# uc-vision/splat-trainer

Hardware: AMD Instinct MI355X
Metric: fwd+bwd Gaussians/s (higher is better)
Workload: dtype f32

## Files before the change

### include/gsplat_hip.h

```cpp
#ifndef GSPLAT_HIP_H
#define GSPLAT_HIP_H

#include <stddef.h>
#include <stdint.h>

#ifdef __cplusplus
extern "C" {
#endif

#define GSR_OK 0
#define GSR_ERR_INVALID_ARGUMENT -1
#define GSR_ERR_WORKSPACE_TOO_SMALL -2
#define GSR_ERR_LAUNCH_FAILED -3
#define GSR_ERR_UNSUPPORTED -4

#define GSR_ROW_FLOATS 16
#define GSR_PARTIAL_FLOATS 12
#define GSR_MAX_FEATURES 16
#define GSR_WIDE_MIN_FEATURES 4

#ifndef GSR_HAVE_RASTER_PARAMS
#define GSR_HAVE_RASTER_PARAMS
typedef struct GsrRasterParamsC {
  float alpha_threshold;
// ... 110 lines not shown
                                     float* d_position, float* d_log_scaling, float* d_rotation, float* d_alpha_logit,
                                     int32_t mode, float* d_colors_out, float* prune_cost_out, float* split_score_out,
                                     float* visibility_out, float* camera_partials, float* d_camera, void* stream);

int gsr_depth_key_range(float near_plane, float far_plane, uint32_t* bias_out, uint32_t* max_key_out);
int gsr_depth_keys(const float* depth, int64_t M, uint32_t bias, uint32_t max_key, uint32_t* keys_out, void* stream);
int gsr_pack_rows(const float* gaussians2d, const float* depth, const float* features, int64_t M, int32_t C,
                  const GsrRasterParamsC* params_host, float* rows_out, float* screen_scale_out, void* stream);
int gsr_pack_rows_wide(const float* gaussians2d, const float* depth, const float* features, int64_t M, int32_t C,
                       const GsrRasterParamsC* params_host, float* rows_out, float* feat_rows_out, float* screen_scale_out,
                       void* stream);
int gsr_tile_count(const float* rows, const uint32_t* order, int64_t M, int32_t W, int32_t H,
                   const GsrRasterParamsC* params_host, uint32_t* count_out, uint32_t* tile_hits_out,
                   const uint32_t* M_dev , void* stream);
#define GSR_TILE_COUNT_OFFSETS_MAX 4194304
size_t gsr_tile_count_offsets_workspace_bytes(int64_t M);
int gsr_tile_count_offsets(const float* rows, const uint32_t* order, int64_t M, int32_t W, int32_t H,
                           const GsrRasterParamsC* params_host, uint32_t* count_out, uint32_t* tile_hits_out,
                           const uint32_t* M_dev, uint32_t* offsets_out, uint32_t* total_dev, uint32_t* overflow_flag,
                           void* workspace, size_t workspace_bytes, void* stream);
int gsr_tile_emit(const float* rows, const uint32_t* order, const uint32_t* offsets, const uint32_t* tile_hits, int64_t M,
                  int32_t W, int32_t H, const GsrRasterParamsC* params_host, uint32_t* keys_out, uint32_t* inst2splat_out,
                  int64_t capacity, const uint32_t* M_dev , void* stream);
int gsr_tile_ranges(const uint32_t* sorted_keys, int64_t O, int32_t num_tiles, uint32_t* tile_range,
                    const uint32_t* O_dev , void* stream);

int gsr_segment_thresholds(int32_t seg_pairs_cfg, int32_t heavy_min_cfg, int64_t O, int32_t num_tiles, int32_t needs_grad,
                           int32_t* seg_pairs_out, int32_t* heavy_min_out);
int64_t gsr_segment_capacity(int64_t O, int32_t O_is_bound, int32_t seg_pairs_cfg, int32_t heavy_min_cfg, int32_t num_tiles,
                             int32_t needs_grad);
int64_t gsr_segment_heavy_capacity(int64_t O, int32_t O_is_bound, int32_t seg_pairs_cfg, int32_t heavy_min_cfg,
                                   int32_t num_tiles, int32_t needs_grad);
int gsr_segment_plan(const uint32_t* tile_range, int32_t num_tiles, int32_t seg_pairs_cfg, int32_t heavy_min_cfg,
                     int32_t needs_grad, int64_t O, const uint32_t* O_dev, int64_t capacity, int64_t heavy_capacity,
                     uint32_t* tile_seg_out, uint32_t* seg_desc_out, uint32_t* seg_total_out, uint32_t* tile_order_out,
                     void* stream);
int gsr_segment_thresholds_wide(int32_t seg_pairs_cfg, int32_t heavy_min_cfg, int64_t O, int32_t num_tiles,
                                int32_t needs_grad, int32_t wide, int32_t* seg_pairs_out, int32_t* heavy_min_out);
int64_t gsr_segment_capacity_wide(int64_t O, int32_t O_is_bound, int32_t seg_pairs_cfg, int32_t heavy_min_cfg,
                                  int32_t num_tiles, int32_t needs_grad, int32_t wide);
int64_t gsr_segment_heavy_capacity_wide(int64_t O, int32_t O_is_bound, int32_t seg_pairs_cfg, int32_t heavy_min_cfg,
                                        int32_t num_tiles, int32_t needs_grad, int32_t wide);
int gsr_segment_plan_wide(const uint32_t* tile_range, int32_t num_tiles, int32_t seg_pairs_cfg, int32_t heavy_min_cfg,
                          int32_t needs_grad, int32_t wide, int64_t O, const uint32_t* O_dev, int64_t capacity,
                          int64_t heavy_capacity, uint32_t* tile_seg_out, uint32_t* seg_desc_out, uint32_t* seg_total_out,
                          uint32_t* tile_order_out, void* stream);
// ... 56 lines not shown
  const float* rotation_xyzw;
  const float* alpha_logit;
  const float* sh_features;
  int64_t N;
  int32_t K;
  int32_t W, H;
  const float* T_camera_world;
  const float* projection;
  const float* camera_pos;
  float near_plane, far_plane;
  GsrRasterParamsC params;
  int32_t want_jacobian;
  int32_t want_median;
  int32_t compute_visibility;
  int32_t needs_grad;
  int32_t seg_pairs, seg_min_pairs;
  int64_t pair_capacity;
  const float* gaussians2d;
  const float* depth;
  const float* features;
  int32_t C;
  const uint32_t* depth_order;
  int32_t feature_table;
} GsrFrameC;
typedef struct GsrFramePlanC {
  int64_t out_bytes, work_bytes;
  int64_t zero_begin, zero_bytes;
  int64_t prune_cost, split_score, counts, tile_range, vis_partial, indexes, rows, screen_scale, jacobian, visibility,
      image, final_T, last, median, count, offsets, vals_a, vals_b, tvals_a, tvals_b, trank_a, trank_b, pair_vis,
      seg_tables, seg_pix, seg_last;
  int64_t seg_capacity, seg_heavy_capacity;
  int64_t cull_ws, sort_ws, scan_ws, tsort_ws, keys_a, keys_b, tile_hits, tkeys_a, tkeys_b;
  int64_t cull_ws_bytes, sort_ws_bytes, scan_ws_bytes, tsort_ws_bytes;
  int64_t feat_rows;
  int64_t seg_col;
} GsrFramePlanC;
typedef struct GsrFrameResultC {
  int64_t order;
  int64_t sorted_inst;
  int64_t sorted_splat;
  GsrSegmentsC segments;
  int32_t has_segments;
} GsrFrameResultC;
int gsr_frame_plan(const GsrFrameC* frame_host, GsrFramePlanC* plan_out_host);
int gsr_frame_forward(const GsrFrameC* frame_host, const GsrFramePlanC* plan_host, void* out_arena, void* work_arena,
                      GsrFrameResultC* result_out_host, uint32_t* counts_host, void* event_counts, void* event_k6_begin,
// ... 296 lines not shown
```

### splat-trainer_amd/csrc/binning.hip

```cpp
#include "gsr_device.h"
#include "gsr_host.h"

namespace {

inline GsrRasterParams to_params(const GsrRasterParamsC* c) {
  GsrRasterParams rp;
  __builtin_memcpy(&rp, c, sizeof(rp));
  return rp;
}

__global__ __launch_bounds__(256) void depth_keys_kernel(const float* __restrict__ depth, int64_t M,
                                                         uint32_t* __restrict__ keys, uint32_t bias, uint32_t max_key) {
  const int64_t m = (int64_t)blockIdx.x * blockDim.x + threadIdx.x;
  if (m >= M) return;
  keys[m] = gsr_depth_key(depth[m], bias, max_key);
}

struct TileHits {
  uint32_t origin;
  uint32_t shape;
  uint32_t lo, hi;
};

__device__ __forceinline__ uint32_t hits_of_large_extent(float u, float v, float A, float B, float C, float qmax, int x0,
                                                         int x1, int y0, int y1, uint32_t* keys, uint32_t* ranks,
                                                         uint32_t o, uint32_t capacity, uint32_t k, int tiles_x,
                                                         int lane) {
  const int nx = x1 - x0, total = nx * (y1 - y0);
  uint32_t n = 0;
  for (int t0 = 0; t0 < total; t0 += 64) {
    const int t = t0 + lane;
    uint32_t hm = 0u;
    int tx = 0, ty = 0;
    if (t < total) {
      ty = y0 + t / nx;
      tx = x0 + t % nx;
      if (gsr_tile_hit(u, v, A, B, C, qmax, tx, ty)) hm = gsr_tile_half_mask(u, v, A, B, C, qmax, tx, ty);
    }
    const uint64_t hit = __ballot(hm != 0u);
    if (keys && hm) {
      const uint32_t at = o + n + (uint32_t)gsr_mbcnt(hit);
      if (at < capacity) {
        keys[at] = (uint32_t)(ty * tiles_x + tx);
        ranks[at] = k | (hm << 30);
      }
    }
    n += (uint32_t)__builtin_popcountll(hit);
  }
  return n;
}

__device__ __forceinline__ float gsr_bcast(float x, int l) {
  return __int_as_float(__builtin_amdgcn_readlane(__float_as_int(x), l));
}

__device__ __forceinline__ uint32_t wave_large_extents(bool large, float u, float v, float A, float B, float C,
                                                       const GsrExtent& e, uint32_t* keys, uint32_t* ranks, uint32_t o,
                                                       uint32_t capacity, uint32_t sid, int tiles_x, int lane) {
  uint32_t mine = 0u;
  uint64_t todo = __ballot(large);
  while (todo) {
    const int l = __builtin_ctzll(todo);
    todo &= todo - 1ull;
    const uint32_t n = hits_of_large_extent(
        gsr_bcast(u, l), gsr_bcast(v, l), gsr_bcast(A, l), gsr_bcast(B, l), gsr_bcast(C, l), gsr_bcast(e.qmax, l),
        __builtin_amdgcn_readlane(e.x0, l), __builtin_amdgcn_readlane(e.x1, l), __builtin_amdgcn_readlane(e.y0, l),
        __builtin_amdgcn_readlane(e.y1, l), keys, ranks, (uint32_t)__builtin_amdgcn_readlane((int)o, l), capacity,
        (uint32_t)__builtin_amdgcn_readlane((int)sid, l), tiles_x, lane);
    if (lane == l) mine = n;
  }
  return mine;
}

__device__ __forceinline__ uint32_t tile_count_one(const float* __restrict__ rows, uint32_t splat,
                                                   int64_t k, bool live, int tiles_x, int tiles_y,
                                                   const GsrRasterParams& rp, TileHits* __restrict__ hits) {
  float2 uv = make_float2(0.f, 0.f), ab = uv, co = uv;
  GsrExtent e;
  e.x0 = e.x1 = e.y0 = e.y1 = 0; e.qmax = 0.f;
  TileHits h;
  h.origin = 0u; h.shape = 0u; h.lo = 0u; h.hi = 0u;
  uint32_t n = 0;
  bool large = false;
  if (live) {
    const int64_t s = splat;
    const float4* r = reinterpret_cast<const float4*>(rows + GSR_ROW_FLOATS * s);
    const float4 r0 = r[0];
    const float4 r1 = r[1];
    uv = make_float2(r0.x, r0.y); ab = make_float2(r0.z, r0.w); co = make_float2(r1.x, r1.y);
    e = gsr_splat_extent(uv.x, uv.y, ab.x, ab.y, co.x, co.y, rp, tiles_x, tiles_y);
    const int nx = e.x1 - e.x0, ny = e.y1 - e.y0;
    h.origin = (uint32_t)e.x0 | ((uint32_t)e.y0 << 16);
    if (nx > 0 && ny > 0) {
      if (nx * ny <= 32) {
        h.shape = (uint32_t)nx | ((uint32_t)ny << 8);
        uint64_t map = 0ull;
        int t = 0;
        for (int ty = e.y0; ty < e.y1; ++ty)
          for (int tx = e.x0; tx < e.x1; ++tx, ++t) {
            const uint64_t hm = gsr_tile_half_mask(uv.x, uv.y, ab.x, ab.y, co.x, e.qmax, tx, ty);
            map |= hm << (2 * t);
            n += hm ? 1u : 0u;
          }
        h.lo = (uint32_t)map; h.hi = (uint32_t)(map >> 32);
      } else {
        h.shape = 1u << 16;
        large = true;
      }
    }
  }
  const uint32_t nl = wave_large_extents(large, uv.x, uv.y, ab.x, ab.y, co.x, e, nullptr, nullptr, 0u, 0u, 0u, tiles_x,
                                         gsr_lane());
  if (large) n = nl;
  if (live) *reinterpret_cast<uint4*>(hits + k) = make_uint4(h.origin, h.shape, h.lo, h.hi);
  return n;
}

__global__ __launch_bounds__(256) void tile_count_kernel(const float* __restrict__ rows,
                                                         const uint32_t* __restrict__ order, int64_t M, int tiles_x,
                                                         int tiles_y, GsrRasterParams rp, uint32_t* __restrict__ count,
                                                         TileHits* __restrict__ hits,
                                                         const uint32_t* __restrict__ M_dev,
                                                         uint32_t* __restrict__ block_sums) {
// ... 34 lines not shown
  before = gsr_wave_sum_u32(before);
  fbefore = gsr_wave_sum(fbefore + (float)sum);
  if (lane == 63) s_wave[w] = incl;
  if (lane == 0) { s_before[w] = before; s_f[w] = fbefore; }
  __syncthreads();
  uint32_t prefix = (s_before[0] + s_before[1]) + (s_before[2] + s_before[3]), total = 0u;
  uint32_t in_block = 0u;
#pragma unroll
  for (int j = 0; j < 4; ++j) {
    if (j < w) in_block += s_wave[j];
    total += s_wave[j];
  }
  if (threadIdx.x == 0 && (s_f[0] + s_f[1]) + (s_f[2] + s_f[3]) >= 2147000000.f) *overflow = 1u;
  uint32_t run = prefix + in_block + incl - sum;
#pragma unroll
  for (int i = 0; i < 16; ++i) {
    if (base + i < n) offsets[base + i] = run;
    run += v[i];
  }
  if (total_out && blockIdx.x == gridDim.x - 1 && threadIdx.x == 0) *total_out = prefix + total;
}


__global__ __launch_bounds__(256) void tile_emit_kernel(const float* __restrict__ rows,
                                                        const uint32_t* __restrict__ order,
                                                        const uint32_t* __restrict__ offsets,
                                                        const TileHits* __restrict__ hits, int64_t M, int tiles_x,
                                                        int tiles_y, GsrRasterParams rp, uint32_t* __restrict__ keys,
                                                        uint32_t* __restrict__ inst2splat, uint32_t capacity,
                                                        const uint32_t* __restrict__ M_dev) {
  const int64_t k = (int64_t)blockIdx.x * blockDim.x + threadIdx.x;
  const bool live = k < M && !(M_dev && k >= (int64_t)*M_dev);
  uint4 hw = make_uint4(0u, 0u, 0u, 0u);
  uint32_t o = 0u, sid = 0u;
  if (live) {
    hw = *reinterpret_cast<const uint4*>(hits + k);
    o = offsets[k];
    sid = order[k];
  }
  const bool large = (hw.y >> 16) != 0u;
  float4 r0 = make_float4(0.f, 0.f, 0.f, 0.f), r1 = r0;
  GsrExtent e;
  e.x0 = e.x1 = e.y0 = e.y1 = 0; e.qmax = 0.f;
  if (large) {
    const float4* r = reinterpret_cast<const float4*>(rows + GSR_ROW_FLOATS * (int64_t)sid);
    r0 = r[0];
    r1 = r[1];
    e = gsr_splat_extent(r0.x, r0.y, r0.z, r0.w, r1.x, r1.y, rp, tiles_x, tiles_y);
  }
  wave_large_extents(large, r0.x, r0.y, r0.z, r0.w, r1.x, e, keys, inst2splat, o, capacity, sid, tiles_x, gsr_lane());
  if (!live || large) return;
  const int nx = (int)(hw.y & 0xFFu), ny = (int)((hw.y >> 8) & 0xFFu);
  const int x0 = (int)(hw.x & 0xFFFFu), y0 = (int)(hw.x >> 16);
  uint64_t map = (uint64_t)hw.z | ((uint64_t)hw.w << 32);
  for (int j = 0; j < ny; ++j)
    for (int i = 0; i < nx; ++i, map >>= 2) {
      const uint32_t hm = (uint32_t)(map & 3ull);
      if (!hm) continue;
      if (o >= capacity) return;
      keys[o] = (uint32_t)((y0 + j) * tiles_x + x0 + i);
      inst2splat[o] = sid | (hm << 30);
// ... 291 lines not shown
int gsr_tile_count_offsets(const float* rows, const uint32_t* order, int64_t M, int32_t W, int32_t H,
                           const GsrRasterParamsC* params_host, uint32_t* count_out, uint32_t* tile_hits_out,
                           const uint32_t* M_dev, uint32_t* offsets_out, uint32_t* total_dev, uint32_t* overflow_flag,
                           void* workspace, size_t workspace_bytes, void* stream_) {
  hipStream_t stream = gsr_stream(stream_);
  if (M < 0 || M > GSR_TILE_COUNT_OFFSETS_MAX || !params_host || W <= 0 || H <= 0) return GSR_ERR_INVALID_ARGUMENT;
  if (params_host->tile_size != 16) return GSR_ERR_UNSUPPORTED;
  if (!total_dev || !overflow_flag) return GSR_ERR_INVALID_ARGUMENT;
  if (M == 0) { hipMemsetAsync(total_dev, 0, sizeof(uint32_t), stream); return GSR_OK; }
  if (!rows || !order || !count_out || !tile_hits_out || !offsets_out) return GSR_ERR_INVALID_ARGUMENT;
  if (!workspace || workspace_bytes < gsr_tile_count_offsets_workspace_bytes(M)) return GSR_ERR_WORKSPACE_TOO_SMALL;
  const auto [tx, ty, num_tiles] = gsr_tiles(W, H);
  if (tx > 0xFFFF || ty > 0xFFFF) return GSR_ERR_UNSUPPORTED;
  uint32_t* sums = reinterpret_cast<uint32_t*>(workspace);
  tile_count_kernel<<<grid_for(M, 256), 256, 0, stream>>>(rows, order, M, tx, ty, to_params(params_host), count_out,
                                                         reinterpret_cast<TileHits*>(tile_hits_out), M_dev, sums);
  GSR_CHECK_LAUNCH();
  offsets_from_sums_kernel<<<grid_for(M, 4096), 256, 0, stream>>>(count_out, (uint32_t)M, sums, offsets_out, total_dev,
                                                                 overflow_flag);
  GSR_CHECK_LAUNCH();
  return GSR_OK;
}

int gsr_tile_emit(const float* rows, const uint32_t* order, const uint32_t* offsets, const uint32_t* tile_hits, int64_t M,
                  int32_t W, int32_t H, const GsrRasterParamsC* params_host, uint32_t* keys_out, uint32_t* inst2splat_out,
                  int64_t capacity, const uint32_t* M_dev, void* stream_) {
  hipStream_t stream = gsr_stream(stream_);
  if (M < 0 || M >= (1ll << 30) || !params_host || W <= 0 || H <= 0) return GSR_ERR_INVALID_ARGUMENT;
  if (capacity < 0 || capacity > 0x7FFFFFFFll) return GSR_ERR_INVALID_ARGUMENT;
  if (params_host->tile_size != 16) return GSR_ERR_UNSUPPORTED;
  if (M == 0) return GSR_OK;
  if (!rows || !order || !offsets || !tile_hits || !keys_out || !inst2splat_out) return GSR_ERR_INVALID_ARGUMENT;
  const auto [tx, ty, num_tiles] = gsr_tiles(W, H);
  tile_emit_kernel<<<grid_for(M, 256), 256, 0, stream>>>(rows, order, offsets, reinterpret_cast<const TileHits*>(tile_hits),
                                                        M, tx, ty, to_params(params_host), keys_out, inst2splat_out,
                                                        (uint32_t)capacity, M_dev);
  GSR_CHECK_LAUNCH();
  return GSR_OK;
}

int gsr_tile_ranges(const uint32_t* sorted_keys, int64_t O, int32_t num_tiles, uint32_t* tile_range,
                    const uint32_t* O_dev, void* stream_) {
  hipStream_t stream = gsr_stream(stream_);
  if (O < 0 || num_tiles <= 0) return GSR_ERR_INVALID_ARGUMENT;
  if (O == 0) return GSR_OK;
  if (!sorted_keys || !tile_range) return GSR_ERR_INVALID_ARGUMENT;
  tile_ranges_kernel<<<grid_for(O, 256), 256, 0, stream>>>(sorted_keys, O, tile_range, O_dev);
  GSR_CHECK_LAUNCH();
  return GSR_OK;
}

int gsr_reduce_visibility(const float* vis_partial, const uint32_t* offsets, const uint32_t* count,
                          const uint32_t* order, int64_t M, float* visibility_out, int64_t capacity,
                          const uint32_t* M_dev, void* stream_) {
  hipStream_t stream = gsr_stream(stream_);
  if (M < 0 || capacity < 0 || capacity > 0x7FFFFFFFll) return GSR_ERR_INVALID_ARGUMENT;
  if (M == 0) return GSR_OK;
  if (!offsets || !count || !visibility_out) return GSR_ERR_INVALID_ARGUMENT;
  reduce_vis_kernel<<<grid_for(M, 256), 256, 0, stream>>>(vis_partial, offsets, count, order, M, visibility_out,
// ... 52 lines not shown
```

### splat-trainer_amd/csrc/frame.hip

```cpp
#include <string.h>

#include "gsr_host.h"

namespace {

inline int64_t align_up(int64_t x, int64_t a = 256) { return (x + a - 1) / a * a; }

struct Cursor {
  int64_t at = 0;
  int64_t take(int64_t bytes) {
    const int64_t o = at;
    at = align_up(at + (bytes > 0 ? bytes : 1));
    return o;
  }
};

inline int tile_bits_of(int num_tiles) {
  int b = 1;
  while ((1 << b) < num_tiles) ++b;
  return b;
}

inline int bit_length(uint32_t v) {
  int b = 0;
// ... 132 lines not shown
    int64_t* indexes = at<int64_t>(out, p->indexes);
    GSR_TRY(gsr_frustum_cull(f->position, N, f->T_camera_world, f->projection, f->W, f->H, f->near_plane, f->far_plane,
                             f->params.margin_px, indexes, M_dev, at<uint8_t>(work, p->cull_ws),
                             (size_t)p->cull_ws_bytes, stream_));
    GSR_TRY(gsr_project_sh_forward(f->position, f->log_scaling, f->rotation_xyzw, f->alpha_logit, f->sh_features, f->K,
                                   indexes, N, f->T_camera_world, f->projection, f->camera_pos, &f->params, rows,
                                   at<float>(out, p->screen_scale), at<float>(out, p->jacobian), M_dev,
                                   keys_a, key_bias, key_max, stream_));
  }
  uint32_t* vals_a = at<uint32_t>(out, p->vals_a);
  uint32_t* vals_b = at<uint32_t>(out, p->vals_b);
  const uint32_t* order = f->depth_order;
  res->order = -1;
  if (!order) {
    const int in_b = gsr_sort_pairs_u32(keys_a, vals_a, at<uint32_t>(work, p->keys_b), vals_b, N, 1, 0, bit_length(key_max),
                                        at<uint8_t>(work, p->sort_ws), (size_t)p->sort_ws_bytes, M_dev, stream_);
    if (in_b < 0) return in_b;
    res->order = in_b == 1 ? p->vals_b : p->vals_a;
    order = in_b == 1 ? vals_b : vals_a;
  }
  uint32_t* count = at<uint32_t>(out, p->count);
  uint32_t* offsets = at<uint32_t>(out, p->offsets);
  uint32_t* hits = at<uint32_t>(work, p->tile_hits);
  if (N <= GSR_TILE_COUNT_OFFSETS_MAX) {
    GSR_TRY(gsr_tile_count_offsets(rows, order, N, f->W, f->H, &f->params, count, hits, M_dev, offsets, O_dev, counts + 2,
                                   at<uint8_t>(work, p->scan_ws), (size_t)p->scan_ws_bytes, stream_));
  } else {
    GSR_TRY(gsr_tile_count(rows, order, N, f->W, f->H, &f->params, count, hits, M_dev, stream_));
    GSR_TRY(gsr_exclusive_scan_u32_checked(count, offsets, N, O_dev, counts + 2, at<uint8_t>(work, p->scan_ws),
                                           (size_t)p->scan_ws_bytes, stream_));
  }
  if (counts_host) {
    if (hipMemcpyAsync(counts_host, counts, 3 * sizeof(uint32_t), hipMemcpyDeviceToHost, stream) != hipSuccess)
      return GSR_ERR_LAUNCH_FAILED;
    if (event_counts && hipEventRecord(reinterpret_cast<hipEvent_t>(event_counts), stream) != hipSuccess)
      return GSR_ERR_LAUNCH_FAILED;
  }
  res->sorted_inst = res->sorted_splat = -1;
  float* image = at<float>(out, p->image);
  if (cap > 0) {
    uint32_t* tkeys_a = at<uint32_t>(work, p->tkeys_a);
    uint32_t* tkeys_b = at<uint32_t>(work, p->tkeys_b);
    uint32_t* tvals_a = at<uint32_t>(out, p->tvals_a);
    uint32_t* tvals_b = at<uint32_t>(out, p->tvals_b);
    uint32_t* trank_a = at<uint32_t>(out, p->trank_a);
    uint32_t* trank_b = at<uint32_t>(out, p->trank_b);
    GSR_TRY(gsr_tile_emit(rows, order, offsets, hits, N, f->W, f->H, &f->params, tkeys_a, trank_a, cap, M_dev, stream_));
    const int sorted = gsr_sort_pairs2_u32(tkeys_a, tvals_a, trank_a, tkeys_b, tvals_b, trank_b, cap, 1, 0, tile_bits_of(T),
                                           at<uint8_t>(work, p->tsort_ws), (size_t)p->tsort_ws_bytes, O_dev, stream_);
    if (sorted < 0) return sorted;
    const bool in_b = sorted == 1;
    res->sorted_inst = in_b ? p->tvals_b : p->tvals_a;
    res->sorted_splat = in_b ? p->trank_b : p->trank_a;
    const uint32_t* sorted_keys = in_b ? tkeys_b : tkeys_a;
    const uint32_t* sorted_inst = in_b ? tvals_b : tvals_a;
    const uint32_t* sorted_splat = in_b ? trank_b : trank_a;
    uint32_t* tile_range = at<uint32_t>(out, p->tile_range);
    GSR_TRY(gsr_tile_ranges(sorted_keys, cap, T, tile_range, O_dev, stream_));
    const GsrSegmentsC* seg = nullptr;
    if (p->seg_capacity > 0) {
      uint32_t* tables = at<uint32_t>(out, p->seg_tables);
      uint32_t* tile_seg = tables;
      uint32_t* seg_desc = tables + 2 * (int64_t)T + p->seg_heavy_capacity;
      uint32_t* seg_total = counts + 3;
      uint32_t* tile_order = seg_desc + 4 * p->seg_capacity;
      GSR_TRY(gsr_segment_plan_wide(tile_range, T, f->seg_pairs, f->seg_min_pairs, f->needs_grad ? 1 : 0,
                                    p->feat_rows >= 0 ? 1 : 0, cap, O_dev, p->seg_capacity, p->seg_heavy_capacity,
                                    tile_seg, seg_desc, seg_total, tile_order, stream_));
      float* pix = at<float>(out, p->seg_pix);
      res->segments.tile_seg = tile_seg;
// ... 106 lines not shown
```

### splat-trainer_amd/csrc/gsr_math.h

```cpp
#pragma once
#include <math.h>

#if defined(__HIPCC__)
#define GSR_HD __host__ __device__ __forceinline__
#else
#define GSR_HD inline
#endif

struct GsrRasterParams {
  float alpha_threshold;
  float clamp_max_alpha;
  float T_eps;
  float q_max;
  float blur;
  int   antialias;
  int   tile_size;
  float margin_px;
};

struct GsrCam {
  float R[9];
  float t[3];
  float fx, fy, cx, cy;
};
// ... 337 lines not shown
GSR_HD GsrExtent gsr_splat_extent(float u, float v, float A, float B, float C, float op,
                                  const GsrRasterParams& rp, int tiles_x, int tiles_y) {
  GsrExtent e;
  e.x0 = e.x1 = e.y0 = e.y1 = 0;
  e.qmax = 0.f;
  if (!(op >= rp.alpha_threshold)) return e;
  float qop = 2.f * logf(op / rp.alpha_threshold) * 1.0001f + 1e-4f;
  float qmax = fminf(rp.q_max * 1.00001f, qop);
  float det = A * C - B * B;
  if (!(det > 0.f)) return e;
  float hx = sqrtf(qmax * C / det) + 1e-3f;
  float hy = sqrtf(qmax * A / det) + 1e-3f;
  const float ts = 16.f;
  float fx0 = floorf((u - hx - 0.5f) / ts), fx1 = floorf((u + hx - 0.5f) / ts) + 1.f;
  float fy0 = floorf((v - hy - 0.5f) / ts), fy1 = floorf((v + hy - 0.5f) / ts) + 1.f;
  e.x0 = (int)fminf(fmaxf(fx0, 0.f), (float)tiles_x);
  e.x1 = (int)fminf(fmaxf(fx1, 0.f), (float)tiles_x);
  e.y0 = (int)fminf(fmaxf(fy0, 0.f), (float)tiles_y);
  e.y1 = (int)fminf(fmaxf(fy1, 0.f), (float)tiles_y);
  e.qmax = qmax;
  return e;
}

GSR_HD float gsr_edge_min_q(float Kf, float Bc, float Kv, float d_fixed, float lo, float hi) {
  float d = -Bc * d_fixed / Kv;
  d = fminf(fmaxf(d, lo), hi);
  return Kf * d_fixed * d_fixed + 2.f * Bc * d_fixed * d + Kv * d * d;
}

GSR_HD bool gsr_rect_hit(float A, float B, float C, float qmax, float rx0, float rx1, float ry0, float ry1) {
  if (rx0 <= 0.f && rx1 >= 0.f && ry0 <= 0.f && ry1 >= 0.f) return true;
  float m = gsr_edge_min_q(A, B, C, rx0, ry0, ry1);
  m = fminf(m, gsr_edge_min_q(A, B, C, rx1, ry0, ry1));
  m = fminf(m, gsr_edge_min_q(C, B, A, ry0, rx0, rx1));
  m = fminf(m, gsr_edge_min_q(C, B, A, ry1, rx0, rx1));
  return m <= qmax;
}

GSR_HD bool gsr_tile_hit(float u, float v, float A, float B, float C, float qmax, int tx, int ty) {
  return gsr_rect_hit(A, B, C, qmax, 16.f * tx + 0.5f - u, 16.f * tx + 15.5f - u, 16.f * ty + 0.5f - v,
                      16.f * ty + 15.5f - v);
}

GSR_HD unsigned gsr_tile_half_mask(float u, float v, float A, float B, float C, float qmax, int tx, int ty) {
  const float rx0 = 16.f * tx + 0.5f - u, rx1 = 16.f * tx + 15.5f - u;
  const float ry = 16.f * ty + 0.5f - v;
  unsigned m = gsr_rect_hit(A, B, C, qmax, rx0, rx1, ry, ry + 7.f) ? 1u : 0u;
  m |= gsr_rect_hit(A, B, C, qmax, rx0, rx1, ry + 8.f, ry + 15.f) ? 2u : 0u;
  return m;
}
```

### splat-trainer_amd/csrc/hostmath_shim.cpp

```cpp
#include "hostmath_shim.h"

#include <stdint.h>
#include <string.h>

#include <algorithm>
#include <utility>
#include <vector>

#include "gsr_math.h"
#include "gsr_bilagrid.h"
#include "gsr_neighbours.h"
#include "gsr_visibility.h"
#include "gsr_filter3d.h"
#include "gsr_sh_fit.h"
#include "gsr_controller.h"
#include "gsr_camera_table.h"
#include "gsr_color.h"
#include "gsr_eval.h"
#include "gsr_histogram.h"
#include "gsr_image.h"
#include "gsr_undistort.h"
#include "gsr_relocate.h"
#include "gsr_fusion.h"
#include "gsr_mesh.h"
// ... 55 lines not shown
    mask[i] = gsr_in_view(cam, pos[3 * i], pos[3 * i + 1], pos[3 * i + 2], W, H, near_p, far_p, margin) ? 1 : 0;
}

void hm_sh_basis(int K, int64_t M, const float* dirs, float* Y) {
  for (int64_t m = 0; m < M; ++m) {
    const float* d = dirs + 3 * m;
    float* y = Y + (int64_t)K * m;
    switch (K) {
      case 1: gsr_sh_basis<1>(d[0], d[1], d[2], y); break;
      case 4: gsr_sh_basis<4>(d[0], d[1], d[2], y); break;
      case 9: gsr_sh_basis<9>(d[0], d[1], d[2], y); break;
      default: gsr_sh_basis<16>(d[0], d[1], d[2], y); break;
    }
  }
}

void hm_tile_hits(const void* params, int64_t M, const float* g2d, int tiles_x, int tiles_y, uint8_t* hits) {
  GsrRasterParams rp;
  memcpy(&rp, params, sizeof(rp));
  const int64_t nt = (int64_t)tiles_x * tiles_y;
  for (int64_t m = 0; m < M; ++m) {
    const float* g = g2d + 6 * m;
    GsrExtent e = gsr_splat_extent(g[0], g[1], g[2], g[3], g[4], g[5], rp, tiles_x, tiles_y);
    for (int ty = e.y0; ty < e.y1; ++ty)
      for (int tx = e.x0; tx < e.x1; ++tx)
        if (gsr_tile_hit(g[0], g[1], g[2], g[3], g[4], e.qmax, tx, ty)) hits[m * nt + ty * tiles_x + tx] = 1;
  }
}

void hm_splat_extent(const void* params, int64_t M, const float* g2d, int tiles_x, int tiles_y, int32_t* extent,
                     float* qmax) {
  GsrRasterParams rp;
  memcpy(&rp, params, sizeof(rp));
  for (int64_t m = 0; m < M; ++m) {
    const float* g = g2d + 6 * m;
    GsrExtent e = gsr_splat_extent(g[0], g[1], g[2], g[3], g[4], g[5], rp, tiles_x, tiles_y);
    int32_t* o = extent + 4 * m;
    o[0] = e.x0; o[1] = e.x1; o[2] = e.y0; o[3] = e.y1;
    qmax[m] = e.qmax;
  }
}

void hm_tile_half_masks(const void* params, int64_t M, const float* g2d, int tiles_x, int tiles_y, uint8_t* masks) {
  GsrRasterParams rp;
  memcpy(&rp, params, sizeof(rp));
  const int64_t nt = (int64_t)tiles_x * tiles_y;
  for (int64_t m = 0; m < M; ++m) {
    const float* g = g2d + 6 * m;
    GsrExtent e = gsr_splat_extent(g[0], g[1], g[2], g[3], g[4], g[5], rp, tiles_x, tiles_y);
    const bool large = (e.x1 - e.x0) * (e.y1 - e.y0) > 32;
    for (int ty = e.y0; ty < e.y1; ++ty)
      for (int tx = e.x0; tx < e.x1; ++tx) {
        if (large && !gsr_tile_hit(g[0], g[1], g[2], g[3], g[4], e.qmax, tx, ty)) continue;
        masks[m * nt + ty * tiles_x + tx] = (uint8_t)gsr_tile_half_mask(g[0], g[1], g[2], g[3], g[4], e.qmax, tx, ty);
      }
  }
}

static void hm_bg_cols(const float* grid, int L, int GH, int GW, int cx, int cy, float* cols) {
  for (int q = 0; q < 4; ++q)
    for (int l = 0; l < L; ++l)
      for (int c = 0; c < GSR_BG_CH; ++c)
        cols[(q * L + l) * GSR_BG_CH + c] = grid[((c * L + l) * GH + cy + (q >> 1)) * GW + cx + (q & 1)];
}

void hm_bilagrid_forward(const float* grid, int L, int GH, int GW, const float* rgb, int H, int W, float* out) {
  float cols[4 * 64 * GSR_BG_CH];
  const float inv_2w = 1.f / (2.f * (float)W), inv_2h = 1.f / (2.f * (float)H);
  for (int i = 0; i < H; ++i)
    for (int j = 0; j < W; ++j) {
      const int cx = gsr_bg_cell(j, W, GW), cy = gsr_bg_cell(i, H, GH);
      hm_bg_cols(grid, L, GH, GW, cx, cy, cols);
      const float* p = rgb + 3 * ((int64_t)i * W + j);
      gsr_bg_pixel_fwd(cols, L, gsr_bg_frac(j, cx, W, GW, inv_2w), gsr_bg_frac(i, cy, H, GH, inv_2h), p[0], p[1], p[2],
                       out + 3 * ((int64_t)i * W + j));
    }
}
// ... 935 lines not shown
```

### splat-trainer_amd/renderer.py

```python
from __future__ import annotations

import ctypes as C
import os
import threading
from typing import Optional, Tuple

import torch

from . import _lib
from ._args import f32
from ._lib import current_stream_ptr as _stream, ptr as _ptr
from .data_types import CameraParams, Gaussians3D, RasterConfig, RenderedPoints, Rendering
from . import sh as _sh
from .sh import evaluate_sh_at

ROW_FLOATS = _lib.CONSTANTS["GSR_ROW_FLOATS"]
PARTIAL_FLOATS = _lib.CONSTANTS["GSR_PARTIAL_FLOATS"]
CAMERA_GRAD_FLOATS = 20


class KernelTimer:

  def __init__(self):
    self.events = {}
    self._open = {}
    self._pool = []

  def reserve(self, n: int):
    for _ in range(n):
      e = torch.cuda.Event(enable_timing=True)
      e.record(_lib.current_stream())
      self._pool.append(e)

  def _event(self):
    e = self._pool.pop() if self._pool else torch.cuda.Event(enable_timing=True)
    e.record(_lib.current_stream())
    return e

  def begin(self, name: str):
    self._open[name] = self._event()
# ... 382 lines not shown

def _vis_out(st: _RasterState, live: bool):
  if live and st.compute_visibility and not st.vis_ready:
    st.vis_ready = True
    return st.visibility
  return None


class _RasterFn(torch.autograd.Function):

  @staticmethod
  def forward(ctx, g2d, feats, depth, st: _RasterState, order):
    g, f, d = f32(g2d), f32(feats), f32(depth).reshape(-1)
    if st.M == 0:
      image = _blank_frame(st, g.device)
    else:
      st.order = order
      frame = _lib.GsrFrameC(
          N=st.M, K=1, W=st.W, H=st.H, near_plane=st.near_far[0], far_plane=st.near_far[1], params=st.params,
          want_median=int(st.want_median), compute_visibility=int(st.compute_visibility),
          needs_grad=int(bool(st.needs_grad)), seg_pairs=st.seg_pairs, seg_min_pairs=st.seg_min,
          gaussians2d=g.data_ptr(), depth=d.data_ptr(), features=f.data_ptr(), C=st.C,
          depth_order=order.data_ptr() if order is not None else None,
          feature_table=int(st.C >= _lib.WIDE_MIN_FEATURES))
      _, _, _, image = _run_frame(frame, st, g.device, st.M, projected=True)
    ctx.st = st
    ctx.in_dtypes = (g2d.dtype, feats.dtype)
    return image

  @staticmethod
  def backward(ctx, d_image):
    st: _RasterState = ctx.st
    dev = d_image.device
    live = st.M > 0 and st.O > 0
    alloc = torch.empty if live else torch.zeros
    d_g2d = alloc(st.M, 6, dtype=torch.float32, device=dev)
    d_feat = alloc(st.M, st.C, dtype=torch.float32, device=dev)
    if live:
      wide = st.C >= _lib.WIDE_MIN_FEATURES
      grows = _composite_backward_wide(st, d_image, d_feat, dev) if wide else _composite_backward_rows(st, d_image, dev)
      _lib.call("gsr_unpack_grad_rows", _ptr(st.rows), _ptr(grows), st.M, st.C, _ptr(d_g2d), None if wide else _ptr(d_feat),
                _ptr(st.prune_cost), _ptr(st.split_score), _ptr(_vis_out(st, live)), _stream())
    return d_g2d.to(ctx.in_dtypes[0]), d_feat.to(ctx.in_dtypes[1]), None, None, None


def _arena_view(typed: torch.Tensor, offset: int, shape) -> torch.Tensor:
  if len(shape) == 1:
# ... 70 lines not shown
  return out, plan, M, image


class _FrameFn(torch.autograd.Function):

  @staticmethod
  def forward(ctx, position, log_scaling, rotation, alpha_logit, feature, T, proj, cam_pos, cull_args, st: _RasterState,
              grad_out, sink, want_jac):
    pos, ls, rot, al = f32(position), f32(log_scaling), f32(rotation), f32(alpha_logit)
    sh, cam = f32(feature), f32(cam_pos)
    N, K, dev = pos.shape[0], sh.shape[2], pos.device
    W, H, near, far, margin = cull_args
    if N == 0:
      st.M = 0
      image = _blank_frame(st, dev)
      indexes, jac = torch.empty(0, dtype=torch.int64, device=dev), None
    else:
      frame = _lib.GsrFrameC(
          position=pos.data_ptr(), log_scaling=ls.data_ptr(), rotation_xyzw=rot.data_ptr(), alpha_logit=al.data_ptr(),
          sh_features=sh.data_ptr(), N=N, K=K, W=W, H=H, T_camera_world=T.data_ptr(), projection=proj.data_ptr(),
          camera_pos=cam.data_ptr(), near_plane=near, far_plane=far, params=st.params,
          want_jacobian=int(bool(want_jac and K > 1)), want_median=int(st.want_median),
          compute_visibility=int(st.compute_visibility), needs_grad=int(bool(st.needs_grad)), seg_pairs=st.seg_pairs,
          seg_min_pairs=st.seg_min, C=3)
      out, plan, M, image = _run_frame(frame, st, dev, N, projected=False)
      indexes = _arena_view(out.view(torch.int64), plan.indexes, (M,))
      jac = _arena_view(out.view(torch.float32), plan.jacobian, (M, 9)) if plan.jacobian >= 0 else None
    rows = st.rows
    ctx.save_for_backward(pos, ls, rot, al, sh, indexes, T, proj, cam)
    ctx.set_materialize_grads(False)
    ctx.st, ctx.jac, ctx.grad_out, ctx.sink = st, jac, grad_out, sink
    ctx.in_dtypes = (position.dtype, log_scaling.dtype, rotation.dtype, alpha_logit.dtype, feature.dtype)
    ctx.mark_non_differentiable(indexes)
    return image, rows[:, 0:6], rows[:, 10:11], indexes

  @staticmethod
  def backward(ctx, d_image, d_g2d, d_depth, _d_indexes):
    pos, ls, rot, al, sh, indexes, T, proj, cam = ctx.saved_tensors
    st: _RasterState = ctx.st
    M, N, K, dev = indexes.shape[0], pos.shape[0], sh.shape[2], pos.device
    go, sink = ctx.grad_out, ctx.sink
    collector = sink.collector if sink is not None else None
    nothing = (None,) * 13
    want_cam = ctx.needs_input_grad[5] or ctx.needs_input_grad[6]
    partials = d_camera = None
    want_sh = sink is not None or ctx.needs_input_grad[4]
    geometry, feature = _sh.gradient_destinations("render_gaussians.backward", N, M, K, go, sink, want_feature=want_sh)
# ... 148 lines not shown
```

Baseline: 579.7 million.

## Fuse offset scan into tile emit kernel and precompute conic reciprocals

For frames up to a size threshold, the exclusive-scan offsets are now computed inside the tile emit kernel. Each block sums the preceding blocks' per-block totals and does a block scan, which removes a separate scan pass and its launches. Separately, the tile-hit tests precompute 1/A and 1/C once per splat and reuse the edge argmin across the two half-tile rects, replacing per-tile divisions. The fused scan makes each block do O(blockIdx) reads of the block sums, a quadratic-ish cost that grows with M.

After: 568.4 million. -2.0%, worse.

```diff
diff --git a/include/gsplat_hip.h b/include/gsplat_hip.h
--- a/include/gsplat_hip.h
+++ b/include/gsplat_hip.h
@@ -156,6 +156,12 @@
 int gsr_tile_emit(const float* rows, const uint32_t* order, const uint32_t* offsets, const uint32_t* tile_hits, int64_t M,
                   int32_t W, int32_t H, const GsrRasterParamsC* params_host, uint32_t* keys_out, uint32_t* inst2splat_out,
                   int64_t capacity, const uint32_t* M_dev , void* stream);
+#define GSR_TILE_EMIT_SCAN_MAX 1048576
+int gsr_tile_bin(const float* rows, const uint32_t* order, int64_t M, int32_t W, int32_t H,
+                 const GsrRasterParamsC* params_host, uint32_t* count_out, uint32_t* tile_hits_out, const uint32_t* M_dev,
+                 uint32_t* offsets_out, uint32_t* total_dev, uint32_t* overflow_flag, uint32_t* keys_out,
+                 uint32_t* inst2splat_out, int64_t capacity, int64_t emit_scan_max, void* workspace,
+                 size_t workspace_bytes, void* stream);
 int gsr_tile_ranges(const uint32_t* sorted_keys, int64_t O, int32_t num_tiles, uint32_t* tile_range,
                     const uint32_t* O_dev , void* stream);
 
@@ -258,6 +264,7 @@
   int32_t C;
   const uint32_t* depth_order;
   int32_t feature_table;
+  int32_t emit_scan_max;
 } GsrFrameC;
 typedef struct GsrFramePlanC {
   int64_t out_bytes, work_bytes;
diff --git a/splat-trainer_amd/csrc/binning.hip b/splat-trainer_amd/csrc/binning.hip
--- a/splat-trainer_amd/csrc/binning.hip
+++ b/splat-trainer_amd/csrc/binning.hip
@@ -22,10 +22,10 @@
   uint32_t lo, hi;
 };
 
-__device__ __forceinline__ uint32_t hits_of_large_extent(float u, float v, float A, float B, float C, float qmax, int x0,
-                                                         int x1, int y0, int y1, uint32_t* keys, uint32_t* ranks,
-                                                         uint32_t o, uint32_t capacity, uint32_t k, int tiles_x,
-                                                         int lane) {
+__device__ __forceinline__ uint32_t hits_of_large_extent(float u, float v, float A, float B, float C,
+                                                         const GsrConicRcp& r, float qmax, int x0, int x1, int y0,
+                                                         int y1, uint32_t* keys, uint32_t* ranks, uint32_t o,
+                                                         uint32_t capacity, uint32_t k, int tiles_x, int lane) {
   const int nx = x1 - x0, total = nx * (y1 - y0);
   uint32_t n = 0;
   for (int t0 = 0; t0 < total; t0 += 64) {
@@ -35,7 +35,7 @@
     if (t < total) {
       ty = y0 + t / nx;
       tx = x0 + t % nx;
-      if (gsr_tile_hit(u, v, A, B, C, qmax, tx, ty)) hm = gsr_tile_half_mask(u, v, A, B, C, qmax, tx, ty);
+      if (gsr_tile_hit(u, v, A, B, C, r, qmax, tx, ty)) hm = gsr_tile_half_mask(u, v, A, B, C, r, qmax, tx, ty);
     }
     const uint64_t hit = __ballot(hm != 0u);
     if (keys && hm) {
@@ -62,8 +62,9 @@
   while (todo) {
     const int l = __builtin_ctzll(todo);
     todo &= todo - 1ull;
+    const float Al = gsr_bcast(A, l), Cl = gsr_bcast(C, l);
     const uint32_t n = hits_of_large_extent(
-        gsr_bcast(u, l), gsr_bcast(v, l), gsr_bcast(A, l), gsr_bcast(B, l), gsr_bcast(C, l), gsr_bcast(e.qmax, l),
+        gsr_bcast(u, l), gsr_bcast(v, l), Al, gsr_bcast(B, l), Cl, gsr_conic_rcp(Al, Cl), gsr_bcast(e.qmax, l),
         __builtin_amdgcn_readlane(e.x0, l), __builtin_amdgcn_readlane(e.x1, l), __builtin_amdgcn_readlane(e.y0, l),
         __builtin_amdgcn_readlane(e.y1, l), keys, ranks, (uint32_t)__builtin_amdgcn_readlane((int)o, l), capacity,
         (uint32_t)__builtin_amdgcn_readlane((int)sid, l), tiles_x, lane);
@@ -94,11 +95,12 @@
     if (nx > 0 && ny > 0) {
       if (nx * ny <= 32) {
         h.shape = (uint32_t)nx | ((uint32_t)ny << 8);
+        const GsrConicRcp rc = gsr_conic_rcp(ab.x, co.x);
         uint64_t map = 0ull;
         int t = 0;
         for (int ty = e.y0; ty < e.y1; ++ty)
           for (int tx = e.x0; tx < e.x1; ++tx, ++t) {
-            const uint64_t hm = gsr_tile_half_mask(uv.x, uv.y, ab.x, ab.y, co.x, e.qmax, tx, ty);
+            const uint64_t hm = gsr_tile_half_mask(uv.x, uv.y, ab.x, ab.y, co.x, rc, e.qmax, tx, ty);
             map |= hm << (2 * t);
             n += hm ? 1u : 0u;
           }
@@ -179,21 +181,49 @@
 }
 
 
+template <bool SCAN>
 __global__ __launch_bounds__(256) void tile_emit_kernel(const float* __restrict__ rows,
                                                         const uint32_t* __restrict__ order,
-                                                        const uint32_t* __restrict__ offsets,
+                                                        std::conditional_t<SCAN, uint32_t, const uint32_t>* __restrict__
+                                                            offsets,
                                                         const TileHits* __restrict__ hits, int64_t M, int tiles_x,
                                                         int tiles_y, GsrRasterParams rp, uint32_t* __restrict__ keys,
                                                         uint32_t* __restrict__ inst2splat, uint32_t capacity,
-                                                        const uint32_t* __restrict__ M_dev) {
+                                                        const uint32_t* __restrict__ M_dev,
+                                                        const uint32_t* __restrict__ count,
+                                                        const uint32_t* __restrict__ sums256,
+                                                        uint32_t* __restrict__ total_out,
+                                                        uint32_t* __restrict__ overflow) {
   const int64_t k = (int64_t)blockIdx.x * blockDim.x + threadIdx.x;
   const bool live = k < M && !(M_dev && k >= (int64_t)*M_dev);
   uint4 hw = make_uint4(0u, 0u, 0u, 0u);
   uint32_t o = 0u, sid = 0u;
   if (live) {
     hw = *reinterpret_cast<const uint4*>(hits + k);
-    o = offsets[k];
+    if constexpr (!SCAN) o = offsets[k];
     sid = order[k];
+  }
+  if constexpr (SCAN) {
+    const uint32_t c = k < M ? count[k] : 0u;
+    uint32_t before = 0u;
+    float fbefore = 0.f;
+    for (uint32_t j = threadIdx.x; j < blockIdx.x; j += 256u) {
+      const uint32_t b = sums256[j];
+      before += b;
+      fbefore += (float)b;
+    }
+    before = gsr_wave_sum_u32(before);
+    fbefore = gsr_wave_sum(fbefore + (float)c);
+    const auto front = gsr_block_handoff(before, fbefore);
+    const uint32_t prefix = (front.a[0] + front.a[1]) + (front.a[2] + front.a[3]);
+    const float shadow = (front.b[0] + front.b[1]) + (front.b[2] + front.b[3]);
+    uint32_t total;
+    o = prefix + gsr_block_scan_excl(c, &total);
+    if (k < M) offsets[k] = o;
+    if (threadIdx.x == 0) {
+      if (shadow >= 2147000000.f) *overflow = 1u;
+      if (blockIdx.x == gridDim.x - 1) *total_out = prefix + total;
+    }
   }
   const bool large = (hw.y >> 16) != 0u;
   float4 r0 = make_float4(0.f, 0.f, 0.f, 0.f), r1 = r0;
@@ -531,6 +561,43 @@
   return GSR_OK;
 }
 
+int gsr_tile_bin(const float* rows, const uint32_t* order, int64_t M, int32_t W, int32_t H,
+                 const GsrRasterParamsC* params_host, uint32_t* count_out, uint32_t* tile_hits_out, const uint32_t* M_dev,
+                 uint32_t* offsets_out, uint32_t* total_dev, uint32_t* overflow_flag, uint32_t* keys_out,
+                 uint32_t* inst2splat_out, int64_t capacity, int64_t emit_scan_max, void* workspace,
+                 size_t workspace_bytes, void* stream_) {
+  hipStream_t stream = gsr_stream(stream_);
+  if (emit_scan_max == 0) emit_scan_max = GSR_TILE_EMIT_SCAN_MAX;
+  if (M > emit_scan_max) {
+    const int rc = gsr_tile_count_offsets(rows, order, M, W, H, params_host, count_out, tile_hits_out, M_dev, offsets_out,
+                                          total_dev, overflow_flag, workspace, workspace_bytes, stream_);
+    if (rc != GSR_OK || M == 0) return rc;
+    return gsr_tile_emit(rows, order, offsets_out, tile_hits_out, M, W, H, params_host, keys_out, inst2splat_out, capacity,
+                         M_dev, stream_);
+  }
+  if (M < 0 || M > GSR_TILE_COUNT_OFFSETS_MAX || !params_host || W <= 0 || H <= 0) return GSR_ERR_INVALID_ARGUMENT;
+  if (capacity < 0 || capacity > 0x7FFFFFFFll) return GSR_ERR_INVALID_ARGUMENT;
+  if (params_host->tile_size != 16) return GSR_ERR_UNSUPPORTED;
+  if (!total_dev || !overflow_flag) return GSR_ERR_INVALID_ARGUMENT;
+  if (M == 0) { hipMemsetAsync(total_dev, 0, sizeof(uint32_t), stream); return GSR_OK; }
+  if (!rows || !order || !count_out || !tile_hits_out || !offsets_out || !keys_out || !inst2splat_out)
+    return GSR_ERR_INVALID_ARGUMENT;
+  if (!workspace || workspace_bytes < gsr_tile_count_offsets_workspace_bytes(M)) return GSR_ERR_WORKSPACE_TOO_SMALL;
+  const auto [tx, ty, num_tiles] = gsr_tiles(W, H);
+  if (tx > 0xFFFF || ty > 0xFFFF) return GSR_ERR_UNSUPPORTED;
+  uint32_t* sums = reinterpret_cast<uint32_t*>(workspace);
+  TileHits* hits = reinterpret_cast<TileHits*>(tile_hits_out);
+  tile_count_kernel<<<grid_for(M, 256), 256, 0, stream>>>(rows, order, M, tx, ty, to_params(params_host), count_out, hits,
+                                                         M_dev, sums);
+  GSR_CHECK_LAUNCH();
+  tile_emit_kernel<true><<<grid_for(M, 256), 256, 0, stream>>>(rows, order, offsets_out, hits, M, tx, ty,
+                                                              to_params(params_host), keys_out, inst2splat_out,
+                                                              (uint32_t)capacity, M_dev, count_out, sums, total_dev,
+                                                              overflow_flag);
+  GSR_CHECK_LAUNCH();
+  return GSR_OK;
+}
+
 int gsr_tile_emit(const float* rows, const uint32_t* order, const uint32_t* offsets, const uint32_t* tile_hits, int64_t M,
                   int32_t W, int32_t H, const GsrRasterParamsC* params_host, uint32_t* keys_out, uint32_t* inst2splat_out,
                   int64_t capacity, const uint32_t* M_dev, void* stream_) {
@@ -541,9 +608,9 @@
   if (M == 0) return GSR_OK;
   if (!rows || !order || !offsets || !tile_hits || !keys_out || !inst2splat_out) return GSR_ERR_INVALID_ARGUMENT;
   const auto [tx, ty, num_tiles] = gsr_tiles(W, H);
-  tile_emit_kernel<<<grid_for(M, 256), 256, 0, stream>>>(rows, order, offsets, reinterpret_cast<const TileHits*>(tile_hits),
-                                                        M, tx, ty, to_params(params_host), keys_out, inst2splat_out,
-                                                        (uint32_t)capacity, M_dev);
+  tile_emit_kernel<false><<<grid_for(M, 256), 256, 0, stream>>>(
+      rows, order, offsets, reinterpret_cast<const TileHits*>(tile_hits), M, tx, ty, to_params(params_host), keys_out,
+      inst2splat_out, (uint32_t)capacity, M_dev, nullptr, nullptr, nullptr, nullptr);
   GSR_CHECK_LAUNCH();
   return GSR_OK;
 }
diff --git a/splat-trainer_amd/csrc/frame.hip b/splat-trainer_amd/csrc/frame.hip
--- a/splat-trainer_amd/csrc/frame.hip
+++ b/splat-trainer_amd/csrc/frame.hip
@@ -178,7 +178,13 @@
   uint32_t* count = at<uint32_t>(out, p->count);
   uint32_t* offsets = at<uint32_t>(out, p->offsets);
   uint32_t* hits = at<uint32_t>(work, p->tile_hits);
-  if (N <= GSR_TILE_COUNT_OFFSETS_MAX) {
+  const int64_t scan_max = f->emit_scan_max == 0 ? (int64_t)GSR_TILE_EMIT_SCAN_MAX : (int64_t)f->emit_scan_max;
+  const bool emit_scans = cap > 0 && N <= scan_max && N <= GSR_TILE_COUNT_OFFSETS_MAX;
+  if (emit_scans) {
+    GSR_TRY(gsr_tile_bin(rows, order, N, f->W, f->H, &f->params, count, hits, M_dev, offsets, O_dev, counts + 2,
+                         at<uint32_t>(work, p->tkeys_a), at<uint32_t>(out, p->trank_a), cap, scan_max,
+                         at<uint8_t>(work, p->scan_ws), (size_t)p->scan_ws_bytes, stream_));
+  } else if (N <= GSR_TILE_COUNT_OFFSETS_MAX) {
     GSR_TRY(gsr_tile_count_offsets(rows, order, N, f->W, f->H, &f->params, count, hits, M_dev, offsets, O_dev, counts + 2,
                                    at<uint8_t>(work, p->scan_ws), (size_t)p->scan_ws_bytes, stream_));
   } else {
@@ -201,7 +207,8 @@
     uint32_t* tvals_b = at<uint32_t>(out, p->tvals_b);
     uint32_t* trank_a = at<uint32_t>(out, p->trank_a);
     uint32_t* trank_b = at<uint32_t>(out, p->trank_b);
-    GSR_TRY(gsr_tile_emit(rows, order, offsets, hits, N, f->W, f->H, &f->params, tkeys_a, trank_a, cap, M_dev, stream_));
+    if (!emit_scans)
+      GSR_TRY(gsr_tile_emit(rows, order, offsets, hits, N, f->W, f->H, &f->params, tkeys_a, trank_a, cap, M_dev, stream_));
     const int sorted = gsr_sort_pairs2_u32(tkeys_a, tvals_a, trank_a, tkeys_b, tvals_b, trank_b, cap, 1, 0, tile_bits_of(T),
                                            at<uint8_t>(work, p->tsort_ws), (size_t)p->tsort_ws_bytes, O_dev, stream_);
     if (sorted < 0) return sorted;
diff --git a/splat-trainer_amd/csrc/gsr_math.h b/splat-trainer_amd/csrc/gsr_math.h
--- a/splat-trainer_amd/csrc/gsr_math.h
+++ b/splat-trainer_amd/csrc/gsr_math.h
@@ -383,30 +383,50 @@
   return e;
 }
 
-GSR_HD float gsr_edge_min_q(float Kf, float Bc, float Kv, float d_fixed, float lo, float hi) {
-  float d = -Bc * d_fixed / Kv;
+struct GsrConicRcp {
+  float rA, rC;
+};
+
+GSR_HD GsrConicRcp gsr_conic_rcp(float A, float C) {
+  GsrConicRcp r;
+  r.rA = 1.0f / A;
+  r.rC = 1.0f / C;
+  return r;
+}
+
+GSR_HD float gsr_edge_argmin(float Bc, float rKv, float d_fixed) { return (-Bc * d_fixed) * rKv; }
+
+GSR_HD float gsr_edge_q_at(float Kf, float Bc, float Kv, float d_fixed, float d, float lo, float hi) {
   d = fminf(fmaxf(d, lo), hi);
   return Kf * d_fixed * d_fixed + 2.f * Bc * d_fixed * d + Kv * d * d;
 }
 
-GSR_HD bool gsr_rect_hit(float A, float B, float C, float qmax, float rx0, float rx1, float ry0, float ry1) {
+GSR_HD float gsr_edge_min_q(float Kf, float Bc, float Kv, float rKv, float d_fixed, float lo, float hi) {
+  return gsr_edge_q_at(Kf, Bc, Kv, d_fixed, gsr_edge_argmin(Bc, rKv, d_fixed), lo, hi);
+}
+
+GSR_HD bool gsr_rect_hit(float A, float B, float C, float rA, float qmax, float rx0, float rx1, float ry0, float ry1,
+                         float dy0, float dy1) {
   if (rx0 <= 0.f && rx1 >= 0.f && ry0 <= 0.f && ry1 >= 0.f) return true;
-  float m = gsr_edge_min_q(A, B, C, rx0, ry0, ry1);
-  m = fminf(m, gsr_edge_min_q(A, B, C, rx1, ry0, ry1));
-  m = fminf(m, gsr_edge_min_q(C, B, A, ry0, rx0, rx1));
-  m = fminf(m, gsr_edge_min_q(C, B, A, ry1, rx0, rx1));
+  float m = gsr_edge_q_at(A, B, C, rx0, dy0, ry0, ry1);
+  m = fminf(m, gsr_edge_q_at(A, B, C, rx1, dy1, ry0, ry1));
+  m = fminf(m, gsr_edge_min_q(C, B, A, rA, ry0, rx0, rx1));
+  m = fminf(m, gsr_edge_min_q(C, B, A, rA, ry1, rx0, rx1));
   return m <= qmax;
 }
 
-GSR_HD bool gsr_tile_hit(float u, float v, float A, float B, float C, float qmax, int tx, int ty) {
-  return gsr_rect_hit(A, B, C, qmax, 16.f * tx + 0.5f - u, 16.f * tx + 15.5f - u, 16.f * ty + 0.5f - v,
-                      16.f * ty + 15.5f - v);
-}
-
-GSR_HD unsigned gsr_tile_half_mask(float u, float v, float A, float B, float C, float qmax, int tx, int ty) {
+GSR_HD bool gsr_tile_hit(float u, float v, float A, float B, float C, const GsrConicRcp& r, float qmax, int tx, int ty) {
+  const float rx0 = 16.f * tx + 0.5f - u, rx1 = 16.f * tx + 15.5f - u;
+  return gsr_rect_hit(A, B, C, r.rA, qmax, rx0, rx1, 16.f * ty + 0.5f - v, 16.f * ty + 15.5f - v,
+                      gsr_edge_argmin(B, r.rC, rx0), gsr_edge_argmin(B, r.rC, rx1));
+}
+
+GSR_HD unsigned gsr_tile_half_mask(float u, float v, float A, float B, float C, const GsrConicRcp& r, float qmax, int tx,
+                                   int ty) {
   const float rx0 = 16.f * tx + 0.5f - u, rx1 = 16.f * tx + 15.5f - u;
   const float ry = 16.f * ty + 0.5f - v;
-  unsigned m = gsr_rect_hit(A, B, C, qmax, rx0, rx1, ry, ry + 7.f) ? 1u : 0u;
-  m |= gsr_rect_hit(A, B, C, qmax, rx0, rx1, ry + 8.f, ry + 15.f) ? 2u : 0u;
+  const float dy0 = gsr_edge_argmin(B, r.rC, rx0), dy1 = gsr_edge_argmin(B, r.rC, rx1);
+  unsigned m = gsr_rect_hit(A, B, C, r.rA, qmax, rx0, rx1, ry, ry + 7.f, dy0, dy1) ? 1u : 0u;
+  m |= gsr_rect_hit(A, B, C, r.rA, qmax, rx0, rx1, ry + 8.f, ry + 15.f, dy0, dy1) ? 2u : 0u;
   return m;
 }
diff --git a/splat-trainer_amd/csrc/hostmath_shim.cpp b/splat-trainer_amd/csrc/hostmath_shim.cpp
--- a/splat-trainer_amd/csrc/hostmath_shim.cpp
+++ b/splat-trainer_amd/csrc/hostmath_shim.cpp
@@ -101,9 +101,10 @@
   for (int64_t m = 0; m < M; ++m) {
     const float* g = g2d + 6 * m;
     GsrExtent e = gsr_splat_extent(g[0], g[1], g[2], g[3], g[4], g[5], rp, tiles_x, tiles_y);
+    const GsrConicRcp r = gsr_conic_rcp(g[2], g[4]);
     for (int ty = e.y0; ty < e.y1; ++ty)
       for (int tx = e.x0; tx < e.x1; ++tx)
-        if (gsr_tile_hit(g[0], g[1], g[2], g[3], g[4], e.qmax, tx, ty)) hits[m * nt + ty * tiles_x + tx] = 1;
+        if (gsr_tile_hit(g[0], g[1], g[2], g[3], g[4], r, e.qmax, tx, ty)) hits[m * nt + ty * tiles_x + tx] = 1;
   }
 }
 
@@ -128,10 +129,12 @@
     const float* g = g2d + 6 * m;
     GsrExtent e = gsr_splat_extent(g[0], g[1], g[2], g[3], g[4], g[5], rp, tiles_x, tiles_y);
     const bool large = (e.x1 - e.x0) * (e.y1 - e.y0) > 32;
+    const GsrConicRcp r = gsr_conic_rcp(g[2], g[4]);
     for (int ty = e.y0; ty < e.y1; ++ty)
       for (int tx = e.x0; tx < e.x1; ++tx) {
-        if (large && !gsr_tile_hit(g[0], g[1], g[2], g[3], g[4], e.qmax, tx, ty)) continue;
-        masks[m * nt + ty * tiles_x + tx] = (uint8_t)gsr_tile_half_mask(g[0], g[1], g[2], g[3], g[4], e.qmax, tx, ty);
+        if (large && !gsr_tile_hit(g[0], g[1], g[2], g[3], g[4], r, e.qmax, tx, ty)) continue;
+        masks[m * nt + ty * tiles_x + tx] =
+            (uint8_t)gsr_tile_half_mask(g[0], g[1], g[2], g[3], g[4], r, e.qmax, tx, ty);
       }
   }
 }
diff --git a/splat-trainer_amd/renderer.py b/splat-trainer_amd/renderer.py
--- a/splat-trainer_amd/renderer.py
+++ b/splat-trainer_amd/renderer.py
@@ -16,6 +16,7 @@
 
 ROW_FLOATS = _lib.CONSTANTS["GSR_ROW_FLOATS"]
 PARTIAL_FLOATS = _lib.CONSTANTS["GSR_PARTIAL_FLOATS"]
+EMIT_SCAN_MAX = 0
 CAMERA_GRAD_FLOATS = 20
 
 
@@ -444,7 +445,7 @@
           needs_grad=int(bool(st.needs_grad)), seg_pairs=st.seg_pairs, seg_min_pairs=st.seg_min,
           gaussians2d=g.data_ptr(), depth=d.data_ptr(), features=f.data_ptr(), C=st.C,
           depth_order=order.data_ptr() if order is not None else None,
-          feature_table=int(st.C >= _lib.WIDE_MIN_FEATURES))
+          feature_table=int(st.C >= _lib.WIDE_MIN_FEATURES), emit_scan_max=EMIT_SCAN_MAX)
       _, _, _, image = _run_frame(frame, st, g.device, st.M, projected=True)
     ctx.st = st
     ctx.in_dtypes = (g2d.dtype, feats.dtype)
@@ -561,7 +562,7 @@
           camera_pos=cam.data_ptr(), near_plane=near, far_plane=far, params=st.params,
           want_jacobian=int(bool(want_jac and K > 1)), want_median=int(st.want_median),
           compute_visibility=int(st.compute_visibility), needs_grad=int(bool(st.needs_grad)), seg_pairs=st.seg_pairs,
-          seg_min_pairs=st.seg_min, C=3)
+          seg_min_pairs=st.seg_min, C=3, emit_scan_max=EMIT_SCAN_MAX)
       out, plan, M, image = _run_frame(frame, st, dev, N, projected=False)
       indexes = _arena_view(out.view(torch.int64), plan.indexes, (M,))
       jac = _arena_view(out.view(torch.float32), plan.jacobian, (M, 9)) if plan.jacobian >= 0 else None
```
